# LambdaLabsML/distributed-training-guide

Hardware: AMD Instinct MI355X
Metric: tokens/sec/GPU for Llama-style causal LM at 1/2/4/8 MI355X; peak HBM per GPU (higher is better)
Workload: dtype bf16; 1 GPU; model=llama-3-8b, global_batch=24, seq_len=1024, parallelism=single

## Files before the change

### distributed_training_guide_amd/_hip/attention_bwd.hip

```cpp
#include "attention_common.h"
#include "launchers.h"

template <int D>
__global__ void __launch_bounds__(256) attn_delta_kernel(
    const short* __restrict__ dout, const short* __restrict__ o,
    float* __restrict__ delta, int B, int S, int Hq) {
  const int grp = threadIdx.x >> 4;
  const int gl = threadIdx.x & 15;
  int64_t nrows = (int64_t)B * S * Hq;
  for (int64_t row = (int64_t)blockIdx.x * 16 + grp; row < nrows;
       row += (int64_t)gridDim.x * 16) {
    const short* dp = dout + row * D;
    const short* op = o + row * D;
    float s = 0.f;
#pragma unroll
    for (int i = gl * 8; i < D; i += 16 * 8) {
      bf16x8 dv = *reinterpret_cast<const bf16x8*>(dp + i);
      bf16x8 ov = *reinterpret_cast<const bf16x8*>(op + i);
#pragma unroll
      for (int j = 0; j < 8; ++j) s += bf2f(dv[j]) * bf2f(ov[j]);
    }
#pragma unroll
    for (int off = 1; off < 16; off <<= 1) s += __shfl_xor(s, off, WAVE);
    if (gl == 0) {
      int h = (int)(row % Hq);
      int64_t bs = row / Hq;
      int sp = (int)(bs % S);
      int b = (int)(bs / S);
      delta[((int64_t)b * Hq + h) * S + sp] = s;
    }
  }
}

template <int D, bool DOC>
__global__ void __launch_bounds__(256, 2) attn_dkdv_kernel(
    const short* __restrict__ dout, const short* __restrict__ q,
    const short* __restrict__ k, const short* __restrict__ v,
    const float* __restrict__ lse, const float* __restrict__ delta,
    short* __restrict__ dk, short* __restrict__ dv, int B, int S, int Hq,
    int Hkv, float scale, const int* __restrict__ doc_end) {
  static_assert(D == 64 || D == 128, "head dim must be 64 or 128");
  __shared__ short q_lds[2][64 * D];
  __shared__ short do_lds[2][64 * D];
  __shared__ __attribute__((aligned(16))) float lse_lds[2][64];
  __shared__ __attribute__((aligned(16))) float del_lds[2][64];

  const int nkt = (S + 63) / 64;
  const int group = Hq / Hkv;

  const GroupBlock gb = xcd_remap(blockIdx.x, B * Hkv, nkt);
  const int b = gb.gid / Hkv;
  const int hkv = gb.gid % Hkv;
  const int kt = gb.within;

  const int tid = threadIdx.x;
  const int wid = tid >> 6;
  const int lane = tid & (WAVE - 1);
  const int l15 = lane & 15;
  const int lg = lane >> 4;

  const int kv0 = kt * 64 + wid * 16;
  constexpr int nd16 = D >> 4, nkc = D >> 5;
  const float c2 = scale * LOG2E;
  const int64_t strideS_q = (int64_t)Hq * D;
  const int64_t strideS_kv = (int64_t)Hkv * D;
  const short* kb = k + ((int64_t)b * S * Hkv + hkv) * D;
  const short* vb = v + ((int64_t)b * S * Hkv + hkv) * D;

  bf16x8 kf[nkc], vf[nkc];
  {
    int key = kv0 + l15;
    int keyc = key < S ? key : S - 1;
    const short* kp = kb + (int64_t)keyc * strideS_kv + lg * 8;
    const short* vp = vb + (int64_t)keyc * strideS_kv + lg * 8;
#pragma unroll
    for (int c = 0; c < nkc; ++c) {
      kf[c] = *reinterpret_cast<const bf16x8*>(kp + c * 32);
      vf[c] = *reinterpret_cast<const bf16x8*>(vp + c * 32);
    }
  }

  f32x4 dkacc[nd16], dvacc[nd16];
#pragma unroll
  for (int i = 0; i < nd16; ++i) {
    dkacc[i] = {0.f, 0.f, 0.f, 0.f};
    dvacc[i] = {0.f, 0.f, 0.f, 0.f};
  }

  const int qstart = kt * 64;
  int dend = S, dend_min = S, qcap = S;
  if (DOC) {
    const int* deb = doc_end + (int64_t)b * S;
    dend = deb[min(kv0 + l15, S - 1)];
    dend_min = deb[min(kv0, S - 1)];
    qcap = min(max(deb[min(qstart + 63, S - 1)], qstart + 1), S);
  }
  const int nqt = (qcap - qstart + 63) / 64;
  const int niter = group * nqt;

  auto stage_qdo = [&](int it, int buf) {
    const int64_t hoff = ((int64_t)b * S * Hq + hkv * group + it / nqt) * D;
    stage_tile_pair<D>(q + hoff, dout + hoff, strideS_q,
                       qstart + (it % nqt) * 64, S, q_lds[buf], do_lds[buf],
                       wid, lane);
  };
  auto stage_lse = [&](int it, int buf) {
    const int hh = hkv * group + it / nqt;
    const int qt = qstart + (it % nqt) * 64;
    if (tid < 64) {
      const float* lseb = lse + ((int64_t)b * Hq + hh) * S;
      int rr = qt + tid < S ? qt + tid : S - 1;
      lse_lds[buf][tid] = lseb[rr] * LOG2E;
    } else if (tid < 128) {
      const float* delb = delta + ((int64_t)b * Hq + hh) * S;
      int rr = qt + tid - 64 < S ? qt + tid - 64 : S - 1;
      del_lds[buf][tid - 64] = delb[rr] * scale;
    }
  };

  stage_qdo(0, 0);
  stage_lse(0, 0);
  __syncthreads();

  for (int it = 0; it < niter; ++it) {
    const int buf = it & 1;
    if (it + 1 < niter) {
      stage_qdo(it + 1, buf ^ 1);
      stage_lse(it + 1, buf ^ 1);
    }

    const int qt = qstart + (it % nqt) * 64;
    const short* ql = q_lds[buf];
    const short* dol = do_lds[buf];

    const int key = kv0 + l15;
    const bool diag = (qt < kt * 64 + 64) || (qt + 63 >= S) ||
                      (DOC && qt + 63 >= dend_min);
    u32x4 pk_p[2], pk_ds[2];
    __builtin_amdgcn_s_setprio(1);
#pragma unroll
    for (int mth = 0; mth < 2; ++mth) {
      const int qra = perm16(2 * mth, l15), qrb = perm16(2 * mth + 1, l15);
      f32x4 sa0 = {0.f, 0.f, 0.f, 0.f}, da0 = {0.f, 0.f, 0.f, 0.f};
      f32x4 sa1 = {0.f, 0.f, 0.f, 0.f}, da1 = {0.f, 0.f, 0.f, 0.f};
#pragma unroll
      for (int c = 0; c < nkc; ++c) {
        bf16x8 qa0 = *reinterpret_cast<const bf16x8*>(
            ql + st_idx(qra, c * 32 + lg * 8));
        bf16x8 qa1 = *reinterpret_cast<const bf16x8*>(
            ql + st_idx(qrb, c * 32 + lg * 8));
        bf16x8 do0 = *reinterpret_cast<const bf16x8*>(
            dol + st_idx(qra, c * 32 + lg * 8));
        bf16x8 do1 = *reinterpret_cast<const bf16x8*>(
            dol + st_idx(qrb, c * 32 + lg * 8));
        sa0 = mfma16(qa0, kf[c], sa0);
        sa1 = mfma16(qa1, kf[c], sa1);
        da0 = mfma16(do0, vf[c], da0);
        da1 = mfma16(do1, vf[c], da1);
      }
#pragma unroll
      for (int half = 0; half < 2; ++half) {
        const int mt = 2 * mth + half;
        const f32x4 sa = half ? sa1 : sa0;
        const f32x4 da = half ? da1 : da0;
        const int qoff = cpos16(mt, lg);
        const f32x4 lse4 =
            *reinterpret_cast<const f32x4*>(&lse_lds[buf][qoff]);
        const f32x4 del4 =
            *reinterpret_cast<const f32x4*>(&del_lds[buf][qoff]);
        float e[4], p[4], ds[4];
#pragma unroll
        for (int r = 0; r < 4; ++r)
          e[r] = __builtin_fmaf(sa[r], c2, -lse4[r]);
        if (diag) {
#pragma unroll
          for (int r = 0; r < 4; ++r) {
            const int qrow = qt + qoff + r;
            if (key > qrow || qrow >= S || key >= S || (DOC && qrow >= dend))
              e[r] = -INFINITY;
          }
        }
#pragma unroll
        for (int r = 0; r < 4; ++r) {
          p[r] = __builtin_amdgcn_exp2f(e[r]);
          ds[r] = p[r] * __builtin_fmaf(da[r], scale, -del4[r]);
        }
        const int kc = mt >> 1, rp = (mt & 1) * 2;
        pk_p[kc][rp + 0] = cvt_pk_bf16(p[0], p[1]);
        pk_p[kc][rp + 1] = cvt_pk_bf16(p[2], p[3]);
        pk_ds[kc][rp + 0] = cvt_pk_bf16(ds[0], ds[1]);
        pk_ds[kc][rp + 1] = cvt_pk_bf16(ds[2], ds[3]);
      }
    }

#pragma unroll
    for (int dt = 0; dt < nd16; ++dt) {
#pragma unroll
      for (int kc = 0; kc < 2; ++kc) {
        bf16x8 dofr = tr16_frag_st(dol, kc * 32 + lg * 8, dt * 16, l15);
        bf16x8 qfr = tr16_frag_st(ql, kc * 32 + lg * 8, dt * 16, l15);
        dvacc[dt] = mfma16(__builtin_bit_cast(bf16x8, pk_p[kc]), dofr,
                           dvacc[dt]);
        dkacc[dt] = mfma16(__builtin_bit_cast(bf16x8, pk_ds[kc]), qfr,
                           dkacc[dt]);
      }
    }
    __builtin_amdgcn_s_setprio(0);
    __syncthreads();
  }

#pragma unroll
  for (int r = 0; r < 4; ++r) {
    int keyw = kv0 + lg * 4 + r;
    if (keyw >= S) continue;
    short* dkp = dk + ((int64_t)b * S * Hkv + (int64_t)keyw * Hkv + hkv) * D;
    short* dvp = dv + ((int64_t)b * S * Hkv + (int64_t)keyw * Hkv + hkv) * D;
#pragma unroll
    for (int dt = 0; dt < nd16; ++dt) {
      dkp[dt * 16 + l15] = f2bf(dkacc[dt][r]);
      dvp[dt * 16 + l15] = f2bf(dvacc[dt][r]);
    }
  }
}

template <int D, bool DOC>
__global__ void __launch_bounds__(256, 2) attn_dq_kernel(
    const short* __restrict__ dout, const short* __restrict__ q,
    const short* __restrict__ k, const short* __restrict__ v,
    const float* __restrict__ lse, const float* __restrict__ delta,
    short* __restrict__ dq, int B, int S, int Hq, int Hkv, float scale,
    const int* __restrict__ doc_start) {
  static_assert(D == 64 || D == 128, "head dim must be 64 or 128");
  __shared__ short k_lds[2][KVBLK * D];
  __shared__ short v_lds[2][KVBLK * D];

  const int ntq = (S + QBLK - 1) / QBLK;
  const int gqa = Hq / Hkv;
  const int bpg = gqa * ntq;

  const GroupBlock gb = xcd_remap(blockIdx.x, B * Hkv, bpg);
  const int b = gb.gid / Hkv;
  const int hkv = gb.gid % Hkv;
  const int h = hkv * gqa + gb.within / ntq;
  const int qtile = gb.within % ntq;

  const int tid = threadIdx.x;
  const int wid = tid >> 6;
  const int lane = tid & (WAVE - 1);
  const int l15 = lane & 15;
  const int lg = lane >> 4;

  const int q0 = qtile * QBLK;
  const int rowb[2] = {qgroup_row(q0, wid, 0), qgroup_row(q0, wid, 1)};
  constexpr int nd16 = D >> 4, nkc = D >> 5;
  const float c2 = scale * LOG2E;
  const int64_t strideS_q = (int64_t)Hq * D;
  const int64_t strideS_kv = (int64_t)Hkv * D;
  const short* qb = q + ((int64_t)b * S * Hq + h) * D;
  const short* dob = dout + ((int64_t)b * S * Hq + h) * D;
  const short* kb = k + ((int64_t)b * S * Hkv + hkv) * D;
  const short* vb = v + ((int64_t)b * S * Hkv + hkv) * D;
  const float* lseb = lse + ((int64_t)b * Hq + h) * S;
  const float* delb = delta + ((int64_t)b * Hq + h) * S;

  bf16x8 qf[2][nkc], dof[2][nkc];
  float lse_r[2], del_r[2];
#pragma unroll
  for (int nq = 0; nq < 2; ++nq) {
    int qrow = rowb[nq] + l15;
    int qrc = qrow < S ? qrow : S - 1;
    const short* qp = qb + (int64_t)qrc * strideS_q + lg * 8;
    const short* dop = dob + (int64_t)qrc * strideS_q + lg * 8;
#pragma unroll
    for (int c = 0; c < nkc; ++c) {
      qf[nq][c] = *reinterpret_cast<const bf16x8*>(qp + c * 32);
      dof[nq][c] = *reinterpret_cast<const bf16x8*>(dop + c * 32);
    }
    lse_r[nq] = lseb[qrc] * LOG2E;
    del_r[nq] = delb[qrc] * scale;
  }

  f32x4 dqacc[nd16][2];
#pragma unroll
  for (int dt = 0; dt < nd16; ++dt)
#pragma unroll
    for (int nq = 0; nq < 2; ++nq) dqacc[dt][nq] = {0.f, 0.f, 0.f, 0.f};

  const int kv_end = min(S, q0 + QBLK);
  const int ntiles = (kv_end + KVBLK - 1) / KVBLK;
  int dstart[2], dsmax[2];
  const int t0 =
      doc_window<DOC>(doc_start, b, S, q0, wid, l15, dstart, dsmax);

  auto stage_kv = [&](int t, int buf) {
    stage_tile_pair<D>(kb, vb, strideS_kv, t * KVBLK, S, k_lds[buf],
                       v_lds[buf], wid, lane);
  };
  stage_kv(t0, 0);
  __syncthreads();

  for (int t = t0; t < ntiles; ++t) {
    const int kv0 = t * KVBLK;
    const int buf = tile_buf(t, t0);
    if (t + 1 < ntiles) stage_kv(t + 1, buf ^ 1);

    {
      const bool smask = (kv_end < kv0 + KVBLK);
      u32x4 pk_ds[2][2];
      const short* kl = k_lds[buf];
      const short* vl = v_lds[buf];
      __builtin_amdgcn_s_setprio(1);
#pragma unroll
      for (int mt = 0; mt < 4; ++mt) {
        const int kr = perm16(mt, l15);
        f32x4 s0 = {0.f, 0.f, 0.f, 0.f}, s1 = {0.f, 0.f, 0.f, 0.f};
        f32x4 d0 = {0.f, 0.f, 0.f, 0.f}, d1 = {0.f, 0.f, 0.f, 0.f};
#pragma unroll
        for (int c = 0; c < nkc; ++c) {
          bf16x8 ka = *reinterpret_cast<const bf16x8*>(
              kl + st_idx(kr, c * 32 + lg * 8));
          bf16x8 va = *reinterpret_cast<const bf16x8*>(
              vl + st_idx(kr, c * 32 + lg * 8));
          s0 = mfma16(ka, qf[0][c], s0);
          d0 = mfma16(va, dof[0][c], d0);
          s1 = mfma16(ka, qf[1][c], s1);
          d1 = mfma16(va, dof[1][c], d1);
        }
        const int koff = cpos16(mt, lg);
        const int kc = mt >> 1, rp = (mt & 1) * 2;
#pragma unroll
        for (int nq = 0; nq < 2; ++nq) {
          const int qrow = rowb[nq] + l15;
          const bool diag = (kv0 + KVBLK - 1 > rowb[nq]) || smask ||
                            (DOC && dsmax[nq] > kv0);
          const f32x4 sv = nq ? s1 : s0;
          const f32x4 dv = nq ? d1 : d0;
          float e[4], ds[4];
#pragma unroll
          for (int r = 0; r < 4; ++r)
            e[r] = __builtin_fmaf(sv[r], c2, -lse_r[nq]);
          if (diag) {
#pragma unroll
            for (int r = 0; r < 4; ++r) {
              const int keyr = kv0 + koff + r;
              if (keyr > qrow || keyr >= S || qrow >= S ||
                  (DOC && keyr < dstart[nq]))
                e[r] = -INFINITY;
            }
          }
#pragma unroll
          for (int r = 0; r < 4; ++r)
            ds[r] = __builtin_amdgcn_exp2f(e[r]) *
                    __builtin_fmaf(dv[r], scale, -del_r[nq]);
          pk_ds[nq][kc][rp + 0] = cvt_pk_bf16(ds[0], ds[1]);
          pk_ds[nq][kc][rp + 1] = cvt_pk_bf16(ds[2], ds[3]);
        }
      }

#pragma unroll
      for (int dt = 0; dt < nd16; ++dt) {
#pragma unroll
        for (int kc = 0; kc < 2; ++kc) {
          bf16x8 kfr = tr16_frag_st(kl, kc * 32 + lg * 8, dt * 16, l15);
          dqacc[dt][0] = mfma16(__builtin_bit_cast(bf16x8, pk_ds[0][kc]),
                                kfr, dqacc[dt][0]);
          dqacc[dt][1] = mfma16(__builtin_bit_cast(bf16x8, pk_ds[1][kc]),
                                kfr, dqacc[dt][1]);
        }
      }
      __builtin_amdgcn_s_setprio(0);
    }
    __syncthreads();
  }

#pragma unroll
  for (int nq = 0; nq < 2; ++nq) {
#pragma unroll
    for (int r = 0; r < 4; ++r) {
      int qrow = rowb[nq] + lg * 4 + r;
      if (qrow >= S) continue;
      short* dqp = dq + ((int64_t)b * S * Hq + (int64_t)qrow * Hq + h) * D;
#pragma unroll
      for (int dt = 0; dt < nd16; ++dt) {
        dqp[dt * 16 + l15] = f2bf(dqacc[dt][nq][r]);
      }
    }
  }
}

namespace {
template <int D, bool DOC>
void bwd_launch(const short* dout, const short* q, const short* k,
                const short* v, const short* o, const float* lse,
                float* delta, short* dq, short* dk, short* dv,
                const int* doc_start, const int* doc_end, int B, int S,
                int Hq, int Hkv, float scale, hipStream_t stream) {
  int64_t nrows = (int64_t)B * S * Hq;
  int64_t dwant = (nrows + 15) / 16;
  int dgrid = (int)(dwant < 2048 ? (dwant < 1 ? 1 : dwant) : 2048);
  hipLaunchKernelGGL(attn_delta_kernel<D>, dim3(dgrid), dim3(256), 0, stream,
                     dout, o, delta, B, S, Hq);
  int nkt = (S + 63) / 64;
  hipLaunchKernelGGL((attn_dkdv_kernel<D, DOC>),
                     dim3((uint32_t)((int64_t)B * Hkv * nkt)), dim3(256), 0,
                     stream, dout, q, k, v, lse, delta, dk, dv, B, S, Hq, Hkv,
                     scale, doc_end);
  int ntq = (S + QBLK - 1) / QBLK;
  hipLaunchKernelGGL((attn_dq_kernel<D, DOC>),
                     dim3((uint32_t)((int64_t)B * Hq * ntq)), dim3(256), 0,
                     stream, dout, q, k, v, lse, delta, dq, B, S, Hq, Hkv,
                     scale, doc_start);
}
}

extern "C" void attn_bwd_launch(const void* dout, const void* q, const void* k,
                                const void* v, const void* o, const float* lse,
                                float* delta, void* dq, void* dk, void* dv,
                                const int* doc_start, const int* doc_end,
                                int B, int S, int Hq, int Hkv, int D,
                                float scale, hipStream_t stream) {
  const bool doc = doc_start != nullptr;
  auto fn = doc ? (D == 64 ? bwd_launch<64, true> : bwd_launch<128, true>)
                : (D == 64 ? bwd_launch<64, false> : bwd_launch<128, false>);
  fn((const short*)dout, (const short*)q, (const short*)k, (const short*)v,
     (const short*)o, lse, delta, (short*)dq, (short*)dk, (short*)dv,
     doc_start, doc_end, B, S, Hq, Hkv, scale, stream);
}
```

### distributed_training_guide_amd/_hip/attention_common.h

```cpp
#pragma once
#include "common.h"

using bf16x8 = s16x8;

constexpr int QBLK = 128;
constexpr int KVBLK = 64;
#define LOG2E 1.4426950408889634f

__device__ __forceinline__ f32x4 mfma16(bf16x8 a, bf16x8 b, f32x4 c) {
  return __builtin_amdgcn_mfma_f32_16x16x32_bf16(a, b, c, 0, 0, 0);
}

template <int D>
__device__ __forceinline__ void stage_tile_pair(
    const short* ga, const short* gb, int64_t stride, int row0, int S,
    short* la, short* lb, int wid, int lane) {
  constexpr int ncw = D >> 5;
#pragma unroll
  for (int i = 0; i < ncw; ++i) {
    const int ch = wid * ncw + i;
    int row = row0 + (ch & 1) * 32 + (lane >> 1);
    if (row >= S) row = S - 1;
    const int64_t goff =
        (int64_t)row * stride + (ch >> 1) * 16 + (lane & 1) * 8;
    __builtin_amdgcn_global_load_lds(
        (const __attribute__((address_space(1))) unsigned int*)(ga + goff),
        (LDS_AS unsigned int*)(la + ch * 512), 16, 0, 0);
    __builtin_amdgcn_global_load_lds(
        (const __attribute__((address_space(1))) unsigned int*)(gb + goff),
        (LDS_AS unsigned int*)(lb + ch * 512), 16, 0, 0);
  }
}

struct GroupBlock {
  int gid;
  int within;
};
__device__ __forceinline__ GroupBlock xcd_remap(int bid, int ngroups,
                                                int bpg) {
  if ((ngroups & 7) == 0)
    return {(bid >> 3) / bpg * 8 + (bid & 7), (bid >> 3) % bpg};
  return {bid / bpg, bid % bpg};
}

__device__ __forceinline__ int qgroup_row(int q0, int wid, int nq) {
  return q0 + nq * 64 + wid * 16;
}

template <bool DOC>
__device__ __forceinline__ int doc_window(const int* doc_start, int b, int S,
                                          int q0, int wid, int l15,
                                          int (&dstart)[2], int (&dsmax)[2]) {
  dstart[0] = dstart[1] = dsmax[0] = dsmax[1] = 0;
  if (!DOC) return 0;
  const int* dsb = doc_start + (int64_t)b * S;
#pragma unroll
  for (int nq = 0; nq < 2; ++nq) {
    dstart[nq] = dsb[min(qgroup_row(q0, wid, nq) + l15, S - 1)];
    dsmax[nq] = dsb[min(qgroup_row(q0, wid, nq) + 15, S - 1)];
  }
  return min(max(dsb[q0], 0), q0) / KVBLK;
}

__device__ __forceinline__ int tile_buf(int t, int t0) { return (t - t0) & 1; }
```

### distributed_training_guide_amd/_hip/attention_fwd.hip

```cpp
#include "attention_common.h"
#include "launchers.h"

template <int D, bool DOC>
__global__ void __launch_bounds__(256, 2) attn_fwd_kernel(
    const short* __restrict__ q, const short* __restrict__ k,
    const short* __restrict__ v, short* __restrict__ o,
    float* __restrict__ lse_out, int B, int S, int Hq, int Hkv, float scale,
    const int* __restrict__ doc_start) {
  static_assert(D == 64 || D == 128, "head dim must be 64 or 128");
  __shared__ short k_lds[2][KVBLK * D];
  __shared__ short v_lds[2][KVBLK * D];

  const int ntq = (S + QBLK - 1) / QBLK;
  const int gqa = Hq / Hkv;
  const int bpg = gqa * ntq;

  const GroupBlock gb = xcd_remap(blockIdx.x, B * Hkv, bpg);
  const int b = gb.gid / Hkv;
  const int hkv = gb.gid % Hkv;
  const int h = hkv * gqa + gb.within / ntq;
  const int qtile = gb.within % ntq;

  const int tid = threadIdx.x;
  const int wid = tid >> 6;
  const int lane = tid & (WAVE - 1);
  const int l15 = lane & 15;
  const int lg = lane >> 4;

  const int q0 = qtile * QBLK;
  const int rowb[2] = {qgroup_row(q0, wid, 0), qgroup_row(q0, wid, 1)};
  constexpr int nd16 = D >> 4;
  constexpr int nkc = D >> 5;
  const int64_t strideS_q = (int64_t)Hq * D;
  const int64_t strideS_kv = (int64_t)Hkv * D;
  const short* qb = q + ((int64_t)b * S * Hq + h) * D;
  const short* kb = k + ((int64_t)b * S * Hkv + hkv) * D;
  const short* vb = v + ((int64_t)b * S * Hkv + hkv) * D;

  bf16x8 qf[2][nkc];
#pragma unroll
  for (int nq = 0; nq < 2; ++nq) {
    int qrow = rowb[nq] + l15;
    if (qrow >= S) qrow = S - 1;
    const short* qp = qb + (int64_t)qrow * strideS_q + lg * 8;
#pragma unroll
    for (int kc = 0; kc < nkc; ++kc)
      qf[nq][kc] = *reinterpret_cast<const bf16x8*>(qp + kc * 32);
  }

  int kperm[4], ckey[4];
#pragma unroll
  for (int mt = 0; mt < 4; ++mt) {
    kperm[mt] = perm16(mt, l15);
    ckey[mt] = cpos16(mt, lg);
  }

  f32x4 oacc[nd16][2];
#pragma unroll
  for (int dt = 0; dt < nd16; ++dt)
#pragma unroll
    for (int nq = 0; nq < 2; ++nq) oacc[dt][nq] = {0.f, 0.f, 0.f, 0.f};
  float mrow[2] = {-INFINITY, -INFINITY};
  float mcrow[2] = {-INFINITY, -INFINITY};
  float lrow[2] = {0.f, 0.f};

  const int kv_end = min(S, q0 + QBLK);
  const int ntiles = (kv_end + KVBLK - 1) / KVBLK;
  const float c = scale * LOG2E;
  int dstart[2], dsmax[2];
  const int t0 =
      doc_window<DOC>(doc_start, b, S, q0, wid, l15, dstart, dsmax);

  auto stage_kv = [&](int t, int buf) {
    stage_tile_pair<D>(kb, vb, strideS_kv, t * KVBLK, S, k_lds[buf],
                       v_lds[buf], wid, lane);
  };
  stage_kv(t0, 0);
  __syncthreads();

  for (int t = t0; t < ntiles; ++t) {
    const int kv0 = t * KVBLK;
    const int buf = tile_buf(t, t0);
    if (t + 1 < ntiles) stage_kv(t + 1, buf ^ 1);


    const short* kl = k_lds[buf];
    f32x4 sfrag[4][2];
    __builtin_amdgcn_s_setprio(1);
#pragma unroll
    for (int mth = 0; mth < 2; ++mth) {
      const int kra = kperm[2 * mth], krb = kperm[2 * mth + 1];
      f32x4 a0 = {0.f, 0.f, 0.f, 0.f}, a1 = {0.f, 0.f, 0.f, 0.f};
      f32x4 b0 = {0.f, 0.f, 0.f, 0.f}, b1 = {0.f, 0.f, 0.f, 0.f};
#pragma unroll
      for (int kc = 0; kc < nkc; ++kc) {
        bf16x8 kfa = *reinterpret_cast<const bf16x8*>(
            kl + st_idx(kra, kc * 32 + lg * 8));
        bf16x8 kfb = *reinterpret_cast<const bf16x8*>(
            kl + st_idx(krb, kc * 32 + lg * 8));
        a0 = mfma16(kfa, qf[0][kc], a0);
        b0 = mfma16(kfb, qf[0][kc], b0);
        a1 = mfma16(kfa, qf[1][kc], a1);
        b1 = mfma16(kfb, qf[1][kc], b1);
      }
      sfrag[2 * mth][0] = a0;
      sfrag[2 * mth][1] = a1;
      sfrag[2 * mth + 1][0] = b0;
      sfrag[2 * mth + 1][1] = b1;
    }
    __builtin_amdgcn_s_setprio(0);

    u32x4 pk[2][2];
    float alpha[2];
#pragma unroll
    for (int nq = 0; nq < 2; ++nq) {
      const int qrow = rowb[nq] + l15;
      const bool need_mask = (kv0 + KVBLK - 1) > rowb[nq] ||
                             kv_end < kv0 + KVBLK ||
                             (DOC && dsmax[nq] > kv0);
      if (need_mask) {
#pragma unroll
        for (int mt = 0; mt < 4; ++mt)
#pragma unroll
          for (int r = 0; r < 4; ++r) {
            int key = kv0 + ckey[mt] + r;
            if (key > qrow || key >= S || (DOC && key < dstart[nq]))
              sfrag[mt][nq][r] = -INFINITY;
          }
      }
      float tmax = -INFINITY;
#pragma unroll
      for (int mt = 0; mt < 4; ++mt) {
        f32x4 s = sfrag[mt][nq];
        tmax = fmaxf(tmax, fmaxf(fmaxf(s[0], s[1]), fmaxf(s[2], s[3])));
      }
      tmax = fmaxf(tmax, __shfl_xor(tmax, 16, WAVE));
      tmax = fmaxf(tmax, __shfl_xor(tmax, 32, WAVE));
      const float mnew = fmaxf(mrow[nq], tmax);
      const float mcn = mnew * c;
      const float mc = (mnew == -INFINITY) ? 0.0f : mcn;
      alpha[nq] = __builtin_amdgcn_exp2f(mcrow[nq] - mc);
      mrow[nq] = mnew;
      mcrow[nq] = mcn;
      float psum = 0.f;
#pragma unroll
      for (int mt = 0; mt < 4; ++mt) {
        f32x4 s = sfrag[mt][nq];
        f32x4 p;
#pragma unroll
        for (int r = 0; r < 4; ++r) {
          p[r] = __builtin_amdgcn_exp2f(__builtin_fmaf(s[r], c, -mc));
          psum += p[r];
        }
        pk[nq][mt >> 1][(mt & 1) * 2 + 0] = cvt_pk_bf16(p[0], p[1]);
        pk[nq][mt >> 1][(mt & 1) * 2 + 1] = cvt_pk_bf16(p[2], p[3]);
      }
      psum += __shfl_xor(psum, 16, WAVE);
      psum += __shfl_xor(psum, 32, WAVE);
      lrow[nq] = lrow[nq] * alpha[nq] + psum;
    }

    const short* vt = v_lds[buf];
    __builtin_amdgcn_s_setprio(1);
#pragma unroll
    for (int dt = 0; dt < nd16; ++dt) {
      bf16x8 va[2];
#pragma unroll
      for (int kc = 0; kc < 2; ++kc)
        va[kc] = tr16_frag_st(vt, kc * 32 + lg * 8, dt * 16, l15);
#pragma unroll
      for (int nq = 0; nq < 2; ++nq) {
        f32x4 acc = oacc[dt][nq];
#pragma unroll
        for (int r = 0; r < 4; ++r) acc[r] *= alpha[nq];
        acc = mfma16(va[0], __builtin_bit_cast(bf16x8, pk[nq][0]), acc);
        acc = mfma16(va[1], __builtin_bit_cast(bf16x8, pk[nq][1]), acc);
        oacc[dt][nq] = acc;
      }
    }
    __builtin_amdgcn_s_setprio(0);
    __syncthreads();
  }

#pragma unroll
  for (int nq = 0; nq < 2; ++nq) {
    const int qrow = rowb[nq] + l15;
    if (qrow >= S) continue;
    const float invl = (lrow[nq] > 0.f) ? 1.0f / lrow[nq] : 0.0f;
    short* op = o + ((int64_t)b * S * Hq + (int64_t)qrow * Hq + h) * D;
#pragma unroll
    for (int dt = 0; dt < nd16; ++dt) {
      s16x4 outv;
#pragma unroll
      for (int r = 0; r < 4; ++r) outv[r] = f2bf(oacc[dt][nq][r] * invl);
      *reinterpret_cast<s16x4*>(op + dt * 16 + lg * 4) = outv;
    }
    if (lg == 0)
      lse_out[((int64_t)b * Hq + h) * S + qrow] =
          mrow[nq] * scale + __logf(fmaxf(lrow[nq], 1e-30f));
  }
}

extern "C" void attn_fwd_launch(const void* q, const void* k, const void* v,
                                void* o, float* lse, const int* doc_start,
                                int B, int S, int Hq, int Hkv, int D,
                                float scale, hipStream_t stream) {
  int ntiles = (S + QBLK - 1) / QBLK;
  int64_t grid = (int64_t)B * Hq * ntiles;
  auto kern = doc_start
                  ? (D == 64 ? attn_fwd_kernel<64, true>
                             : attn_fwd_kernel<128, true>)
                  : (D == 64 ? attn_fwd_kernel<64, false>
                             : attn_fwd_kernel<128, false>);
  hipLaunchKernelGGL(kern, dim3((uint32_t)grid), dim3(256), 0, stream,
                     (const short*)q, (const short*)k, (const short*)v,
                     (short*)o, lse, B, S, Hq, Hkv, scale, doc_start);
}
```

### distributed_training_guide_amd/_hip/bindings.cpp

```cpp
#include <torch/extension.h>
#include <c10/hip/HIPException.h>
#include <c10/hip/HIPStream.h>
#include <hip/hip_runtime.h>

#include "launchers.h"

namespace {

inline hipStream_t cur_stream() {
  return c10::hip::getCurrentHIPStream().stream();
}

#define CHECK_BF16_CONTIG(t)                                          \
  TORCH_CHECK((t).is_cuda(), #t " must be on the GPU");               \
  TORCH_CHECK((t).dtype() == torch::kBFloat16, #t " must be bf16");   \
  TORCH_CHECK((t).is_contiguous(), #t " must be contiguous")

#define CHECK_ROPE_TABLES(cos, sin, x, D)                                  \
  TORCH_CHECK((D) % 2 == 0, "rope head dim must be even");                 \
  TORCH_CHECK((cos).is_cuda() && (cos).device() == (x).device() &&         \
                  (sin).is_cuda() && (sin).device() == (x).device(),       \
              "rope tables must be on " #x "'s device");                   \
  TORCH_CHECK((cos).dtype() == torch::kFloat &&                            \
                  (sin).dtype() == torch::kFloat,                          \
// ... 375 lines not shown
                  lse.numel() == nrows,
              "lse must be a contiguous f32 [B*S_out] on the logits' device");
  const float* sp = nullptr;
  if (scale_t.has_value()) {
    TORCH_CHECK(scale_t->dtype() == torch::kFloat && scale_t->is_cuda() &&
                scale_t->numel() == 1, "scale_t must be a cuda f32 scalar");
    sp = scale_t->data_ptr<float>();
  }
  auto dlogits = (S_out == S) ? torch::empty_like(logits)
                              : torch::zeros_like(logits);
  ce_bwd_launch(logits.data_ptr(), labels.data_ptr<int64_t>(),
                lse.data_ptr<float>(), dlogits.data_ptr(), (float)scale, sp,
                nrows, S, (int)S_out, V, vocab_start, ignore_index,
                sharded ? 1 : 0, cur_stream());
  return dlogits;
}

void adamw_step(torch::Tensor descs, int64_t nchunks, double lr, double beta1,
                double beta2, double eps, double wd, int64_t step) {
  TORCH_CHECK(descs.is_cuda() && descs.dtype() == torch::kLong &&
              descs.is_contiguous());
  const float bc1 = 1.0f - std::pow((float)beta1, (float)step);
  const float bc2 = 1.0f - std::pow((float)beta2, (float)step);
  adamw_launch(descs.data_ptr(), (int)nchunks, (float)lr, (float)beta1,
               (float)beta2, (float)eps, (float)wd, 1.0f / bc1, 1.0f / bc2,
               cur_stream());
}

#define CHECK_DESCS(descs, nchunks)                                        \
  TORCH_CHECK((descs).is_cuda() && (descs).dtype() == torch::kLong &&      \
              (descs).is_contiguous());                                    \
  TORCH_CHECK((nchunks) >= 0 && (descs).numel() >= 7 * (nchunks),          \
              "descriptor table shorter than nchunks")

#define CHECK_SQ_TOTAL(t, descs)                                           \
  TORCH_CHECK((t).is_cuda() && (t).dtype() == torch::kFloat &&             \
              (t).numel() == 1 && (t).device() == (descs).device(),        \
              #t " must be a cuda f32 scalar on the descriptors' device")

void adamw_step_clipped(torch::Tensor descs, int64_t nchunks, double lr,
                        double beta1, double beta2, double eps, double wd,
                        int64_t step, torch::Tensor sq_total,
                        double max_norm) {
  CHECK_DESCS(descs, nchunks);
  CHECK_SQ_TOTAL(sq_total, descs);
  const float bc1 = 1.0f - std::pow((float)beta1, (float)step);
  const float bc2 = 1.0f - std::pow((float)beta2, (float)step);
  adamw_launch_clipped(descs.data_ptr(), (int)nchunks, (float)lr,
                       (float)beta1, (float)beta2, (float)eps, (float)wd,
                       1.0f / bc1, 1.0f / bc2, sq_total.data_ptr<float>(),
                       (float)max_norm, cur_stream());
}

void grad_sqsum(torch::Tensor descs, int64_t nchunks, torch::Tensor partials,
                torch::Tensor out, int64_t slot) {
  CHECK_DESCS(descs, nchunks);
  TORCH_CHECK(partials.is_cuda() && partials.dtype() == torch::kFloat &&
              partials.is_contiguous() && partials.numel() >= nchunks &&
              partials.device() == descs.device(),
              "partials must be a cuda f32 buffer of >= nchunks elements");
  TORCH_CHECK(out.is_cuda() && out.dtype() == torch::kFloat &&
              out.is_contiguous() && out.device() == descs.device() &&
              slot >= 0 && slot < out.numel(),
              "out must be a cuda f32 buffer holding `slot`");
  grad_sqsum_launch(descs.data_ptr(), (int)nchunks,
                    partials.data_ptr<float>(), out.data_ptr<float>(),
                    (int)slot, cur_stream());
}

void grad_scale_(torch::Tensor descs, int64_t nchunks, torch::Tensor sq_total,
                 double max_norm) {
  CHECK_DESCS(descs, nchunks);
  CHECK_SQ_TOTAL(sq_total, descs);
  grad_scale_launch(descs.data_ptr(), (int)nchunks,
                    sq_total.data_ptr<float>(), (float)max_norm,
                    cur_stream());
}

inline void fp8_check_input(const torch::Tensor& x) {
  CHECK_BF16_CONTIG(x);
  TORCH_CHECK(x.dim() == 2, "fp8 quantisation expects a 2-D [R, C] tensor");
  TORCH_CHECK(x.size(0) > 0 && x.size(1) > 0 && x.size(0) % 16 == 0 &&
                  x.size(1) % 16 == 0,
              "fp8 quantisation requires R and C to be positive multiples "
              "of 16, got [", x.size(0), ", ", x.size(1), "]");
  TORCH_CHECK(x.size(0) <= INT32_MAX && x.size(1) <= INT32_MAX,
              "fp8 quantisation: R and C must fit in int32");
  TORCH_CHECK(reinterpret_cast<uintptr_t>(x.data_ptr()) % 16 == 0,
              "fp8 quantisation requires a 16-byte aligned tensor");
}

torch::Tensor fp8_amax_scale(torch::Tensor x) {
  fp8_check_input(x);
  auto partials = torch::empty({(int64_t)fp8_amax_blocks(x.numel())},
                               x.options().dtype(torch::kInt));
  auto scales = torch::empty({2}, x.options().dtype(torch::kFloat));
  fp8_amax_scale_launch(x.data_ptr(), x.numel(), partials.data_ptr(),
                        scales.data_ptr<float>(), cur_stream());
  C10_HIP_KERNEL_LAUNCH_CHECK();
  return scales;
}

std::tuple<c10::optional<torch::Tensor>, c10::optional<torch::Tensor>>
fp8_cast_transpose(torch::Tensor x, torch::Tensor scale, bool rowwise,
                   bool transposed) {
  fp8_check_input(x);
  TORCH_CHECK(rowwise || transposed,
              "fp8_cast_transpose: ask for at least one output");
  TORCH_CHECK(scale.is_cuda() && scale.device() == x.device(),
              "scale must be on x's device");
  TORCH_CHECK(scale.dtype() == torch::kFloat && scale.numel() == 1,
              "scale must be a single f32 value");
  const int64_t R = x.size(0), C = x.size(1);
  auto opts = x.options().dtype(at::kFloat8_e4m3fn);
  c10::optional<torch::Tensor> q, qt;
  if (rowwise) q = torch::empty({R, C}, opts);
  if (transposed) qt = torch::empty({C, R}, opts);
  fp8_cast_transpose_launch(x.data_ptr(), scale.data_ptr<float>(),
                            q ? q->data_ptr() : nullptr,
                            qt ? qt->data_ptr() : nullptr, (int)R, (int)C,
                            cur_stream());
  C10_HIP_KERNEL_LAUNCH_CHECK();
  return {q, qt};
}

#define CHECK_DOC_TABLE(t, q)                                              \
  TORCH_CHECK((t).is_cuda() && (t).device() == (q).device(),               \
              #t " must be on q's device");                                \
  TORCH_CHECK((t).dtype() == torch::kInt, #t " must be int32");            \
  TORCH_CHECK((t).is_contiguous(), #t " must be contiguous");              \
  TORCH_CHECK((t).dim() == 2 && (t).size(0) == (q).size(0) &&              \
              (t).size(1) == (q).size(1), #t " must be [B,S]")

struct AttnDims {
  int B, S, Hq, Hkv, D;
};

AttnDims attn_check_qkv(const torch::Tensor& q, const torch::Tensor& k,
                        const torch::Tensor& v) {
  CHECK_BF16_CONTIG(q);
  CHECK_BF16_CONTIG(k);
  CHECK_BF16_CONTIG(v);
  TORCH_CHECK(q.dim() == 4, "q must be [B,S,Hq,D]");
  TORCH_CHECK(k.dim() == 4 && k.size(0) == q.size(0) &&
                  k.size(1) == q.size(1) && k.size(3) == q.size(3),
              "k must be [B,S,Hkv,D]");
  TORCH_CHECK(v.sizes() == k.sizes(), "v must be [B,S,Hkv,D]");
  TORCH_CHECK(k.device() == q.device() && v.device() == q.device(),
              "k and v must be on q's device");
  const AttnDims d = {(int)q.size(0), (int)q.size(1), (int)q.size(2),
                      (int)k.size(2), (int)q.size(3)};
  TORCH_CHECK(d.Hq % d.Hkv == 0, "GQA requires Hq % Hkv == 0");
  TORCH_CHECK(d.D == 64 || d.D == 128, "head dim must be 64 or 128");
  return d;
}

std::vector<torch::Tensor> attn_fwd_impl(const torch::Tensor& q,
                                         const torch::Tensor& k,
                                         const torch::Tensor& v,
                                         const torch::Tensor& doc_start,
                                         double scale) {
  const AttnDims d = attn_check_qkv(q, k, v);
  const bool doc = doc_start.defined();
  if (doc) {
    CHECK_DOC_TABLE(doc_start, q);
  }
  auto o = torch::empty_like(q);
  auto lse = torch::empty({(int64_t)d.B, (int64_t)d.Hq, (int64_t)d.S},
                          q.options().dtype(torch::kFloat));
  attn_fwd_launch(q.data_ptr(), k.data_ptr(), v.data_ptr(), o.data_ptr(),
                  lse.data_ptr<float>(),
                  doc ? doc_start.data_ptr<int>() : nullptr, d.B, d.S, d.Hq,
                  d.Hkv, d.D, (float)scale, cur_stream());
  return {o, lse};
}

std::vector<torch::Tensor> attn_bwd_impl(
    const torch::Tensor& dout, const torch::Tensor& q, const torch::Tensor& k,
    const torch::Tensor& v, const torch::Tensor& o, const torch::Tensor& lse,
    const torch::Tensor& doc_start, const torch::Tensor& doc_end,
    double scale) {
  const AttnDims d = attn_check_qkv(q, k, v);
  CHECK_BF16_CONTIG(dout);
  CHECK_BF16_CONTIG(o);
  TORCH_CHECK(dout.sizes() == q.sizes() && o.sizes() == q.sizes(),
              "dout and o must be [B,S,Hq,D] like q");
  TORCH_CHECK(lse.is_cuda() && lse.dtype() == torch::kFloat &&
                  lse.is_contiguous() && lse.dim() == 3 &&
                  lse.size(0) == d.B && lse.size(1) == d.Hq &&
                  lse.size(2) == d.S,
              "lse must be a contiguous cuda f32 [B,Hq,S]");
  TORCH_CHECK(dout.device() == q.device() && o.device() == q.device() &&
                  lse.device() == q.device(),
              "dout, o and lse must be on q's device");
  const bool doc = doc_start.defined();
  if (doc) {
    CHECK_DOC_TABLE(doc_start, q);
    CHECK_DOC_TABLE(doc_end, q);
  }
  auto dq = torch::empty_like(q);
  auto dk = torch::empty_like(k);
  auto dv = torch::empty_like(v);
  auto delta = torch::empty({(int64_t)d.B, (int64_t)d.Hq, (int64_t)d.S},
                            q.options().dtype(torch::kFloat));
  attn_bwd_launch(dout.data_ptr(), q.data_ptr(), k.data_ptr(), v.data_ptr(),
                  o.data_ptr(), lse.data_ptr<float>(),
                  delta.data_ptr<float>(), dq.data_ptr(), dk.data_ptr(),
                  dv.data_ptr(), doc ? doc_start.data_ptr<int>() : nullptr,
                  doc ? doc_end.data_ptr<int>() : nullptr, d.B, d.S, d.Hq,
                  d.Hkv, d.D, (float)scale, cur_stream());
  return {dq, dk, dv};
}

std::vector<torch::Tensor> attn_fwd(torch::Tensor q, torch::Tensor k,
                                    torch::Tensor v, double scale) {
  return attn_fwd_impl(q, k, v, torch::Tensor(), scale);
}
std::vector<torch::Tensor> attn_fwd_doc(torch::Tensor q, torch::Tensor k,
                                        torch::Tensor v,
                                        torch::Tensor doc_start,
                                        double scale) {
  return attn_fwd_impl(q, k, v, doc_start, scale);
}
std::vector<torch::Tensor> attn_bwd(torch::Tensor dout, torch::Tensor q,
                                    torch::Tensor k, torch::Tensor v,
                                    torch::Tensor o, torch::Tensor lse,
                                    double scale) {
  return attn_bwd_impl(dout, q, k, v, o, lse, torch::Tensor(), torch::Tensor(),
                       scale);
}
std::vector<torch::Tensor> attn_bwd_doc(torch::Tensor dout, torch::Tensor q,
                                        torch::Tensor k, torch::Tensor v,
                                        torch::Tensor o, torch::Tensor lse,
                                        torch::Tensor doc_start,
                                        torch::Tensor doc_end, double scale) {
  return attn_bwd_impl(dout, q, k, v, o, lse, doc_start, doc_end, scale);
}

}

PYBIND11_MODULE(TORCH_EXTENSION_NAME, m) {
  m.def("rmsnorm_fwd", &rmsnorm_fwd);
  m.def("rmsnorm_bwd", &rmsnorm_bwd);
  m.def("rope", &rope);
  m.def("add_rmsnorm_fwd", &add_rmsnorm_fwd);
  m.def("add_rmsnorm_bwd", &add_rmsnorm_bwd);
  m.def("qkv_rope_fwd", &qkv_rope_fwd);
  m.def("qkv_rope_bwd", &qkv_rope_bwd);
  m.def("silu_mul_fwd", &silu_mul_fwd);
  m.def("silu_mul_bwd", &silu_mul_bwd);
  m.def("embedding_fwd", &embedding_fwd);
  m.def("embedding_bwd", &embedding_bwd);
  m.def("layernorm_fwd", &layernorm_fwd);
  m.def("layernorm_bwd", &layernorm_bwd);
  m.def("gelu_fwd", &gelu_fwd);
  m.def("gelu_bwd", &gelu_bwd);
  m.def("ce_fwd", &ce_fwd);
  m.def("ce_fwd_sharded", &ce_fwd_sharded);
  m.def("ce_bwd", &ce_bwd, py::arg("logits"), py::arg("labels"),
        py::arg("lse"), py::arg("scale"), py::arg("S_out"),
        py::arg("vocab_start"), py::arg("ignore_index"),
        py::arg("sharded"), py::arg("scale_t") = c10::nullopt);
  m.def("adamw_step", &adamw_step);
  m.def("adamw_step_clipped", &adamw_step_clipped);
  m.def("grad_sqsum", &grad_sqsum);
  m.def("grad_scale_", &grad_scale_);
  m.def("fp8_amax_scale", &fp8_amax_scale);
  m.def("fp8_cast_transpose", &fp8_cast_transpose);
  m.def("attn_fwd", &attn_fwd);
  m.def("attn_bwd", &attn_bwd);
  m.def("attn_fwd_doc", &attn_fwd_doc);
  m.def("attn_bwd_doc", &attn_bwd_doc);
}
```

Measured before the change: 23820 tokens/s.

## Rework attention kernels: buffer loads, LDS-staged stores, unrolled double-buffering, diagonal peel

Switches tile staging from global_load_lds to buffer_load_lds with a buffer resource, and stages output tiles (O, dK, dV, dQ) through LDS so they go to global memory as coalesced 16-byte row writes instead of scattered 2-byte or 8-byte stores. Unrolls the double-buffered loops by two with named buffers, removing the dynamic buffer indexing. Peels the last diagonal KV tile so the fully masked lower query group skips its MFMAs. Reverses the q-tile order so the heavy causal tiles are scheduled first. It adds extra LDS round trips and syncs at the epilogue, and a 2^31-byte limit check for the buffer offsets.

```diff
diff --git a/distributed_training_guide_amd/_hip/attention_bwd.hip b/distributed_training_guide_amd/_hip/attention_bwd.hip
--- a/distributed_training_guide_amd/_hip/attention_bwd.hip
+++ b/distributed_training_guide_amd/_hip/attention_bwd.hip
@@ -1,3 +1,5 @@
+#include <type_traits>
+
 #include "attention_common.h"
 #include "launchers.h"
 
@@ -40,10 +42,10 @@
     short* __restrict__ dk, short* __restrict__ dv, int B, int S, int Hq,
     int Hkv, float scale, const int* __restrict__ doc_end) {
   static_assert(D == 64 || D == 128, "head dim must be 64 or 128");
-  __shared__ short q_lds[2][64 * D];
-  __shared__ short do_lds[2][64 * D];
-  __shared__ __attribute__((aligned(16))) float lse_lds[2][64];
-  __shared__ __attribute__((aligned(16))) float del_lds[2][64];
+  __shared__ short q_lds0[64 * D], q_lds1[64 * D];
+  __shared__ short do_lds0[64 * D], do_lds1[64 * D];
+  __shared__ __attribute__((aligned(16))) float lse_lds0[64], lse_lds1[64];
+  __shared__ __attribute__((aligned(16))) float del_lds0[64], del_lds1[64];
 
   const int nkt = (S + 63) / 64;
   const int group = Hq / Hkv;
@@ -98,40 +100,45 @@
   const int nqt = (qcap - qstart + 63) / 64;
   const int niter = group * nqt;
 
-  auto stage_qdo = [&](int it, int buf) {
+  auto stage_qdo = [&](int it, short* qn, short* don) {
     const int64_t hoff = ((int64_t)b * S * Hq + hkv * group + it / nqt) * D;
     stage_tile_pair<D>(q + hoff, dout + hoff, strideS_q,
-                       qstart + (it % nqt) * 64, S, q_lds[buf], do_lds[buf],
-                       wid, lane);
+                       qstart + (it % nqt) * 64, S, qn, don, wid, lane);
   };
-  auto stage_lse = [&](int it, int buf) {
+  auto load_row = [&](int it) {
     const int hh = hkv * group + it / nqt;
     const int qt = qstart + (it % nqt) * 64;
+    float val = 0.f;
     if (tid < 64) {
       const float* lseb = lse + ((int64_t)b * Hq + hh) * S;
       int rr = qt + tid < S ? qt + tid : S - 1;
-      lse_lds[buf][tid] = lseb[rr] * LOG2E;
+      val = lseb[rr];
     } else if (tid < 128) {
       const float* delb = delta + ((int64_t)b * Hq + hh) * S;
       int rr = qt + tid - 64 < S ? qt + tid - 64 : S - 1;
-      del_lds[buf][tid - 64] = delb[rr] * scale;
-    }
+      val = delb[rr];
+    }
+    return val;
   };
-
-  stage_qdo(0, 0);
-  stage_lse(0, 0);
-  __syncthreads();
-
-  for (int it = 0; it < niter; ++it) {
-    const int buf = it & 1;
-    if (it + 1 < niter) {
-      stage_qdo(it + 1, buf ^ 1);
-      stage_lse(it + 1, buf ^ 1);
+  auto write_row = [&](float val, float* lsen, float* deln) {
+    if (tid < 64) {
+      lsen[tid] = val * LOG2E;
+    } else if (tid < 128) {
+      deln[tid - 64] = val * scale;
+    }
+  };
+
+  auto tile = [&](int it, const short* ql, const short* dol,
+                  const float* lsel, const float* dell, short* qn, short* don,
+                  float* lsen, float* deln) __attribute__((always_inline)) {
+    const bool more = it + 1 < niter;
+    float rowv = 0.f;
+    if (more) {
+      rowv = load_row(it + 1);
+      stage_qdo(it + 1, qn, don);
     }
 
     const int qt = qstart + (it % nqt) * 64;
-    const short* ql = q_lds[buf];
-    const short* dol = do_lds[buf];
 
     const int key = kv0 + l15;
     const bool diag = (qt < kt * 64 + 64) || (qt + 63 >= S) ||
@@ -164,10 +171,8 @@
         const f32x4 sa = half ? sa1 : sa0;
         const f32x4 da = half ? da1 : da0;
         const int qoff = cpos16(mt, lg);
-        const f32x4 lse4 =
-            *reinterpret_cast<const f32x4*>(&lse_lds[buf][qoff]);
-        const f32x4 del4 =
-            *reinterpret_cast<const f32x4*>(&del_lds[buf][qoff]);
+        const f32x4 lse4 = *reinterpret_cast<const f32x4*>(&lsel[qoff]);
+        const f32x4 del4 = *reinterpret_cast<const f32x4*>(&dell[qoff]);
         float e[4], p[4], ds[4];
 #pragma unroll
         for (int r = 0; r < 4; ++r)
@@ -206,21 +211,43 @@
       }
     }
     __builtin_amdgcn_s_setprio(0);
+    if (more) write_row(rowv, lsen, deln);
+  };
+
+  stage_qdo(0, q_lds0, do_lds0);
+  write_row(load_row(0), lse_lds0, del_lds0);
+  __syncthreads();
+
+  int it = 0;
+  do {
+    tile(it, q_lds0, do_lds0, lse_lds0, del_lds0, q_lds1, do_lds1, lse_lds1,
+         del_lds1);
     __syncthreads();
-  }
-
-#pragma unroll
-  for (int r = 0; r < 4; ++r) {
-    int keyw = kv0 + lg * 4 + r;
-    if (keyw >= S) continue;
-    short* dkp = dk + ((int64_t)b * S * Hkv + (int64_t)keyw * Hkv + hkv) * D;
-    short* dvp = dv + ((int64_t)b * S * Hkv + (int64_t)keyw * Hkv + hkv) * D;
-#pragma unroll
-    for (int dt = 0; dt < nd16; ++dt) {
-      dkp[dt * 16 + l15] = f2bf(dkacc[dt][r]);
-      dvp[dt * 16 + l15] = f2bf(dvacc[dt][r]);
-    }
-  }
+    if (it + 1 < niter) {
+      tile(it + 1, q_lds1, do_lds1, lse_lds1, del_lds1, q_lds0, do_lds0,
+           lse_lds0, del_lds0);
+      __syncthreads();
+    }
+    it += 2;
+  } while (it < niter);
+
+  short* kimg = q_lds0 + wid * 16 * D;
+  short* vimg = do_lds0 + wid * 16 * D;
+#pragma unroll
+  for (int dt = 0; dt < nd16; ++dt) {
+    s16x4 kv4, vv4;
+#pragma unroll
+    for (int r = 0; r < 4; ++r) {
+      kv4[r] = f2bf(dkacc[dt][r]);
+      vv4[r] = f2bf(dvacc[dt][r]);
+    }
+    frag_to_rows<D, false>(kimg, dt, kv4, l15, lg);
+    frag_to_rows<D, false>(vimg, dt, vv4, l15, lg);
+  }
+  __syncthreads();
+  const int64_t kvoff = ((int64_t)b * S * Hkv + hkv) * D;
+  rows_to_global<D>(kimg, dk + kvoff, strideS_kv, kv0, S, lane);
+  rows_to_global<D>(vimg, dv + kvoff, strideS_kv, kv0, S, lane);
 }
 
 template <int D, bool DOC>
@@ -231,8 +258,8 @@
     short* __restrict__ dq, int B, int S, int Hq, int Hkv, float scale,
     const int* __restrict__ doc_start) {
   static_assert(D == 64 || D == 128, "head dim must be 64 or 128");
-  __shared__ short k_lds[2][KVBLK * D];
-  __shared__ short v_lds[2][KVBLK * D];
+  __shared__ short k_lds0[KVBLK * D], k_lds1[KVBLK * D];
+  __shared__ short v_lds0[KVBLK * D], v_lds1[KVBLK * D];
 
   const int ntq = (S + QBLK - 1) / QBLK;
   const int gqa = Hq / Hkv;
@@ -242,7 +269,7 @@
   const int b = gb.gid / Hkv;
   const int hkv = gb.gid % Hkv;
   const int h = hkv * gqa + gb.within / ntq;
-  const int qtile = gb.within % ntq;
+  const int qtile = ntq - 1 - gb.within % ntq;
 
   const int tid = threadIdx.x;
   const int wid = tid >> 6;
@@ -292,23 +319,19 @@
   const int t0 =
       doc_window<DOC>(doc_start, b, S, q0, wid, l15, dstart, dsmax);
 
-  auto stage_kv = [&](int t, int buf) {
-    stage_tile_pair<D>(kb, vb, strideS_kv, t * KVBLK, S, k_lds[buf],
-                       v_lds[buf], wid, lane);
-  };
-  stage_kv(t0, 0);
-  __syncthreads();
-
-  for (int t = t0; t < ntiles; ++t) {
+  const bool peel = (ntiles - 1) * KVBLK >= q0 + 64;
+  const int nmain = ntiles - (peel ? 1 : 0);
+
+  auto tile = [&](auto g0c, int t, const short* kl, const short* vl,
+                  short* kn, short* vn) __attribute__((always_inline)) {
+    constexpr int G0 = decltype(g0c)::value;
     const int kv0 = t * KVBLK;
-    const int buf = tile_buf(t, t0);
-    if (t + 1 < ntiles) stage_kv(t + 1, buf ^ 1);
-
+    if (t + 1 < ntiles)
+      stage_tile_pair<D>(kb, vb, strideS_kv, (t + 1) * KVBLK, S, kn, vn, wid,
+                         lane);
     {
       const bool smask = (kv_end < kv0 + KVBLK);
       u32x4 pk_ds[2][2];
-      const short* kl = k_lds[buf];
-      const short* vl = v_lds[buf];
       __builtin_amdgcn_s_setprio(1);
 #pragma unroll
       for (int mt = 0; mt < 4; ++mt) {
@@ -321,15 +344,17 @@
               kl + st_idx(kr, c * 32 + lg * 8));
           bf16x8 va = *reinterpret_cast<const bf16x8*>(
               vl + st_idx(kr, c * 32 + lg * 8));
-          s0 = mfma16(ka, qf[0][c], s0);
-          d0 = mfma16(va, dof[0][c], d0);
+          if constexpr (G0 == 0) {
+            s0 = mfma16(ka, qf[0][c], s0);
+            d0 = mfma16(va, dof[0][c], d0);
+          }
           s1 = mfma16(ka, qf[1][c], s1);
           d1 = mfma16(va, dof[1][c], d1);
         }
         const int koff = cpos16(mt, lg);
         const int kc = mt >> 1, rp = (mt & 1) * 2;
 #pragma unroll
-        for (int nq = 0; nq < 2; ++nq) {
+        for (int nq = G0; nq < 2; ++nq) {
           const int qrow = rowb[nq] + l15;
           const bool diag = (kv0 + KVBLK - 1 > rowb[nq]) || smask ||
                             (DOC && dsmax[nq] > kv0);
@@ -362,30 +387,57 @@
 #pragma unroll
         for (int kc = 0; kc < 2; ++kc) {
           bf16x8 kfr = tr16_frag_st(kl, kc * 32 + lg * 8, dt * 16, l15);
-          dqacc[dt][0] = mfma16(__builtin_bit_cast(bf16x8, pk_ds[0][kc]),
-                                kfr, dqacc[dt][0]);
+          if constexpr (G0 == 0)
+            dqacc[dt][0] = mfma16(__builtin_bit_cast(bf16x8, pk_ds[0][kc]),
+                                  kfr, dqacc[dt][0]);
           dqacc[dt][1] = mfma16(__builtin_bit_cast(bf16x8, pk_ds[1][kc]),
                                 kfr, dqacc[dt][1]);
         }
       }
       __builtin_amdgcn_s_setprio(0);
     }
+  };
+  constexpr std::integral_constant<int, 0> both{};
+  constexpr std::integral_constant<int, 1> upper{};
+
+  stage_tile_pair<D>(kb, vb, strideS_kv, t0 * KVBLK, S, k_lds0, v_lds0, wid,
+                     lane);
+  __syncthreads();
+
+  int t = t0;
+  do {
+    tile(both, t, k_lds0, v_lds0, k_lds1, v_lds1);
     __syncthreads();
-  }
-
-#pragma unroll
-  for (int nq = 0; nq < 2; ++nq) {
-#pragma unroll
-    for (int r = 0; r < 4; ++r) {
-      int qrow = rowb[nq] + lg * 4 + r;
-      if (qrow >= S) continue;
-      short* dqp = dq + ((int64_t)b * S * Hq + (int64_t)qrow * Hq + h) * D;
-#pragma unroll
-      for (int dt = 0; dt < nd16; ++dt) {
-        dqp[dt * 16 + l15] = f2bf(dqacc[dt][nq][r]);
-      }
-    }
-  }
+    if (t + 1 < nmain) {
+      tile(both, t + 1, k_lds1, v_lds1, k_lds0, v_lds0);
+      __syncthreads();
+    }
+    t += 2;
+  } while (t < nmain);
+  if (peel) {
+    if (tile_buf(ntiles - 1, t0))
+      tile(upper, ntiles - 1, k_lds1, v_lds1, k_lds0, v_lds0);
+    else
+      tile(upper, ntiles - 1, k_lds0, v_lds0, k_lds1, v_lds1);
+    __syncthreads();
+  }
+
+  const int el = wave_lane();
+  short* img[2] = {k_lds0 + wid * 16 * D, k_lds1 + wid * 16 * D};
+#pragma unroll
+  for (int nq = 0; nq < 2; ++nq)
+#pragma unroll
+    for (int dt = 0; dt < nd16; ++dt) {
+      s16x4 outv;
+#pragma unroll
+      for (int r = 0; r < 4; ++r) outv[r] = f2bf(dqacc[dt][nq][r]);
+      frag_to_rows<D, false>(img[nq], dt, outv, el & 15, el >> 4);
+    }
+  __syncthreads();
+  short* dqb = dq + ((int64_t)b * S * Hq + h) * D;
+#pragma unroll
+  for (int nq = 0; nq < 2; ++nq)
+    rows_to_global<D>(img[nq], dqb, strideS_q, rowb[nq], S, el);
 }
 
 namespace {
diff --git a/distributed_training_guide_amd/_hip/attention_common.h b/distributed_training_guide_amd/_hip/attention_common.h
--- a/distributed_training_guide_amd/_hip/attention_common.h
+++ b/distributed_training_guide_amd/_hip/attention_common.h
@@ -11,24 +11,32 @@
   return __builtin_amdgcn_mfma_f32_16x16x32_bf16(a, b, c, 0, 0, 0);
 }
 
+__device__ __forceinline__ __amdgpu_buffer_rsrc_t tile_rsrc(const short* base,
+                                                            int64_t stride,
+                                                            int S, int D) {
+  return __builtin_amdgcn_make_buffer_rsrc(
+      const_cast<short*>(base), 0, (int)(((S - 1) * stride + D) * 2),
+      0x00020000);
+}
+
 template <int D>
 __device__ __forceinline__ void stage_tile_pair(
     const short* ga, const short* gb, int64_t stride, int row0, int S,
     short* la, short* lb, int wid, int lane) {
   constexpr int ncw = D >> 5;
+  const __amdgpu_buffer_rsrc_t ra = tile_rsrc(ga, stride, S, D);
+  const __amdgpu_buffer_rsrc_t rb = tile_rsrc(gb, stride, S, D);
 #pragma unroll
   for (int i = 0; i < ncw; ++i) {
     const int ch = wid * ncw + i;
     int row = row0 + (ch & 1) * 32 + (lane >> 1);
     if (row >= S) row = S - 1;
-    const int64_t goff =
-        (int64_t)row * stride + (ch >> 1) * 16 + (lane & 1) * 8;
-    __builtin_amdgcn_global_load_lds(
-        (const __attribute__((address_space(1))) unsigned int*)(ga + goff),
-        (LDS_AS unsigned int*)(la + ch * 512), 16, 0, 0);
-    __builtin_amdgcn_global_load_lds(
-        (const __attribute__((address_space(1))) unsigned int*)(gb + goff),
-        (LDS_AS unsigned int*)(lb + ch * 512), 16, 0, 0);
+    const int boff =
+        (row * (int)stride + (ch >> 1) * 16 + (lane & 1) * 8) * 2;
+    __builtin_amdgcn_raw_ptr_buffer_load_lds(
+        ra, (LDS_AS void*)(la + ch * 512), 16, boff, 0, 0, 0);
+    __builtin_amdgcn_raw_ptr_buffer_load_lds(
+        rb, (LDS_AS void*)(lb + ch * 512), 16, boff, 0, 0, 0);
   }
 }
 
@@ -63,3 +71,45 @@
 }
 
 __device__ __forceinline__ int tile_buf(int t, int t0) { return (t - t0) & 1; }
+
+template <int D>
+__device__ __forceinline__ int row_sw(int row) {
+  return D == 128 ? ((row ^ (row >> 2)) & 7) : (((row >> 1) ^ (row >> 2)) & 3);
+}
+
+template <int D, bool ROW_L15>
+__device__ __forceinline__ void frag_to_rows(short* img, int dt, s16x4 v,
+                                             int l15, int lg) {
+  if (ROW_L15) {
+    *reinterpret_cast<s16x4*>(img + l15 * D + ((dt ^ row_sw<D>(l15)) << 4) +
+                              lg * 4) = v;
+  } else {
+#pragma unroll
+    for (int r = 0; r < 4; ++r) {
+      const int row = lg * 4 + r;
+      img[row * D + ((dt ^ row_sw<D>(row)) << 4) + l15] = v[r];
+    }
+  }
+}
+
+__device__ __forceinline__ int wave_lane() {
+  return __builtin_amdgcn_mbcnt_hi(~0u, __builtin_amdgcn_mbcnt_lo(~0u, 0u));
+}
+
+template <int D>
+__device__ __forceinline__ void rows_to_global(const short* img, short* gp,
+                                               int64_t stride, int row0, int S,
+                                               int lane) {
+  constexpr int lpr = D >> 3;
+  constexpr int rpi = WAVE / lpr;
+  const int c8 = lane % lpr;
+#pragma unroll
+  for (int i = 0; i < 16 / rpi; ++i) {
+    const int row = i * rpi + lane / lpr;
+    const s16x8 val = *reinterpret_cast<const s16x8*>(
+        img + row * D + (((c8 >> 1) ^ row_sw<D>(row)) << 4) + (c8 & 1) * 8);
+    if (row0 + row < S)
+      *reinterpret_cast<s16x8*>(gp + (int64_t)(row0 + row) * stride + c8 * 8) =
+          val;
+  }
+}
diff --git a/distributed_training_guide_amd/_hip/attention_fwd.hip b/distributed_training_guide_amd/_hip/attention_fwd.hip
--- a/distributed_training_guide_amd/_hip/attention_fwd.hip
+++ b/distributed_training_guide_amd/_hip/attention_fwd.hip
@@ -1,3 +1,5 @@
+#include <type_traits>
+
 #include "attention_common.h"
 #include "launchers.h"
 
@@ -8,8 +10,8 @@
     float* __restrict__ lse_out, int B, int S, int Hq, int Hkv, float scale,
     const int* __restrict__ doc_start) {
   static_assert(D == 64 || D == 128, "head dim must be 64 or 128");
-  __shared__ short k_lds[2][KVBLK * D];
-  __shared__ short v_lds[2][KVBLK * D];
+  __shared__ short k_lds0[KVBLK * D], k_lds1[KVBLK * D];
+  __shared__ short v_lds0[KVBLK * D], v_lds1[KVBLK * D];
 
   const int ntq = (S + QBLK - 1) / QBLK;
   const int gqa = Hq / Hkv;
@@ -19,7 +21,7 @@
   const int b = gb.gid / Hkv;
   const int hkv = gb.gid % Hkv;
   const int h = hkv * gqa + gb.within / ntq;
-  const int qtile = gb.within % ntq;
+  const int qtile = ntq - 1 - gb.within % ntq;
 
   const int tid = threadIdx.x;
   const int wid = tid >> 6;
@@ -71,20 +73,17 @@
   const int t0 =
       doc_window<DOC>(doc_start, b, S, q0, wid, l15, dstart, dsmax);
 
-  auto stage_kv = [&](int t, int buf) {
-    stage_tile_pair<D>(kb, vb, strideS_kv, t * KVBLK, S, k_lds[buf],
-                       v_lds[buf], wid, lane);
-  };
-  stage_kv(t0, 0);
-  __syncthreads();
-
-  for (int t = t0; t < ntiles; ++t) {
+  const bool peel = (ntiles - 1) * KVBLK >= q0 + 64;
+  const int nmain = ntiles - (peel ? 1 : 0);
+
+  auto tile = [&](auto g0c, int t, const short* kl, const short* vt,
+                  short* kn, short* vn) __attribute__((always_inline)) {
+    constexpr int G0 = decltype(g0c)::value;
     const int kv0 = t * KVBLK;
-    const int buf = tile_buf(t, t0);
-    if (t + 1 < ntiles) stage_kv(t + 1, buf ^ 1);
-
-
-    const short* kl = k_lds[buf];
+    if (t + 1 < ntiles)
+      stage_tile_pair<D>(kb, vb, strideS_kv, (t + 1) * KVBLK, S, kn, vn, wid,
+                         lane);
+
     f32x4 sfrag[4][2];
     __builtin_amdgcn_s_setprio(1);
 #pragma unroll
@@ -98,8 +97,10 @@
             kl + st_idx(kra, kc * 32 + lg * 8));
         bf16x8 kfb = *reinterpret_cast<const bf16x8*>(
             kl + st_idx(krb, kc * 32 + lg * 8));
-        a0 = mfma16(kfa, qf[0][kc], a0);
-        b0 = mfma16(kfb, qf[0][kc], b0);
+        if constexpr (G0 == 0) {
+          a0 = mfma16(kfa, qf[0][kc], a0);
+          b0 = mfma16(kfb, qf[0][kc], b0);
+        }
         a1 = mfma16(kfa, qf[1][kc], a1);
         b1 = mfma16(kfb, qf[1][kc], b1);
       }
@@ -113,7 +114,7 @@
     u32x4 pk[2][2];
     float alpha[2];
 #pragma unroll
-    for (int nq = 0; nq < 2; ++nq) {
+    for (int nq = G0; nq < 2; ++nq) {
       const int qrow = rowb[nq] + l15;
       const bool need_mask = (kv0 + KVBLK - 1) > rowb[nq] ||
                              kv_end < kv0 + KVBLK ||
@@ -160,7 +161,6 @@
       lrow[nq] = lrow[nq] * alpha[nq] + psum;
     }
 
-    const short* vt = v_lds[buf];
     __builtin_amdgcn_s_setprio(1);
 #pragma unroll
     for (int dt = 0; dt < nd16; ++dt) {
@@ -169,7 +169,7 @@
       for (int kc = 0; kc < 2; ++kc)
         va[kc] = tr16_frag_st(vt, kc * 32 + lg * 8, dt * 16, l15);
 #pragma unroll
-      for (int nq = 0; nq < 2; ++nq) {
+      for (int nq = G0; nq < 2; ++nq) {
         f32x4 acc = oacc[dt][nq];
 #pragma unroll
         for (int r = 0; r < 4; ++r) acc[r] *= alpha[nq];
@@ -179,26 +179,53 @@
       }
     }
     __builtin_amdgcn_s_setprio(0);
+  };
+  constexpr std::integral_constant<int, 0> both{};
+  constexpr std::integral_constant<int, 1> upper{};
+
+  stage_tile_pair<D>(kb, vb, strideS_kv, t0 * KVBLK, S, k_lds0, v_lds0, wid,
+                     lane);
+  __syncthreads();
+
+  int t = t0;
+  do {
+    tile(both, t, k_lds0, v_lds0, k_lds1, v_lds1);
     __syncthreads();
-  }
-
+    if (t + 1 < nmain) {
+      tile(both, t + 1, k_lds1, v_lds1, k_lds0, v_lds0);
+      __syncthreads();
+    }
+    t += 2;
+  } while (t < nmain);
+  if (peel) {
+    if (tile_buf(ntiles - 1, t0))
+      tile(upper, ntiles - 1, k_lds1, v_lds1, k_lds0, v_lds0);
+    else
+      tile(upper, ntiles - 1, k_lds0, v_lds0, k_lds1, v_lds1);
+    __syncthreads();
+  }
+
+  short* img[2] = {k_lds0 + wid * 16 * D, k_lds1 + wid * 16 * D};
 #pragma unroll
   for (int nq = 0; nq < 2; ++nq) {
     const int qrow = rowb[nq] + l15;
-    if (qrow >= S) continue;
     const float invl = (lrow[nq] > 0.f) ? 1.0f / lrow[nq] : 0.0f;
-    short* op = o + ((int64_t)b * S * Hq + (int64_t)qrow * Hq + h) * D;
 #pragma unroll
     for (int dt = 0; dt < nd16; ++dt) {
       s16x4 outv;
 #pragma unroll
       for (int r = 0; r < 4; ++r) outv[r] = f2bf(oacc[dt][nq][r] * invl);
-      *reinterpret_cast<s16x4*>(op + dt * 16 + lg * 4) = outv;
-    }
-    if (lg == 0)
+      frag_to_rows<D, true>(img[nq], dt, outv, l15, lg);
+    }
+    if (lg == 0 && qrow < S)
       lse_out[((int64_t)b * Hq + h) * S + qrow] =
           mrow[nq] * scale + __logf(fmaxf(lrow[nq], 1e-30f));
   }
+  __syncthreads();
+  short* ob = o + ((int64_t)b * S * Hq + h) * D;
+#pragma unroll
+  for (int nq = 0; nq < 2; ++nq)
+    rows_to_global<D>(img[nq], ob, strideS_q, rowb[nq], S, lane);
 }
 
 extern "C" void attn_fwd_launch(const void* q, const void* k, const void* v,
diff --git a/distributed_training_guide_amd/_hip/bindings.cpp b/distributed_training_guide_amd/_hip/bindings.cpp
--- a/distributed_training_guide_amd/_hip/bindings.cpp
+++ b/distributed_training_guide_amd/_hip/bindings.cpp
@@ -551,6 +551,8 @@
                       (int)k.size(2), (int)q.size(3)};
   TORCH_CHECK(d.Hq % d.Hkv == 0, "GQA requires Hq % Hkv == 0");
   TORCH_CHECK(d.D == 64 || d.D == 128, "head dim must be 64 or 128");
+  TORCH_CHECK(q.size(1) * q.size(2) * q.size(3) * 2 < (int64_t{1} << 31),
+              "attention needs S * Hq * D * 2 < 2^31 bytes per batch row");
   return d;
 }
 
```

Result: no change. 23970 tokens/s, median of 6 (+0.6%).
